# zkemail/halo2-regex

Hardware: AMD Instinct MI355X
Metric: DFA witness rows/sec (higher is better)
Workload: dtype u8

## Files before the change

### halo2_regex_amd/csrc/hrx_api.cpp

```cpp
#include <fstream>
#include <sstream>

#include "hrx_ctx.hpp"
#include "hrx_fr.h"
#include "hrx_host_walk.hpp"
#include "hrx_lane.h"

using namespace hrx;

static thread_local std::string g_err;
int hrx::set_last_error(int code, const std::string &msg) {
    g_err = msg;
    return code;
}

namespace hrx {
uint32_t debug_flags_from_env() {
    const char *dbg = std::getenv("HRX_DEBUG_FLAGS");
    return dbg ? ((uint32_t)std::strtoul(dbg, nullptr, 0) & kDbgHonoured) : 0u;
}
bool match_via_rows_from_env() {
    const char *dbg = std::getenv("HRX_DEBUG_FLAGS");
    return dbg && (std::strtoull(dbg, nullptr, 0) & kDbgMatchViaRows) != 0;
}
// ... 142 lines not shown
    return table_endpoint_rows(defs->s, d, rows3, cap_rows);
}


int hrx_device_count(int *count) {
    if (!count) return fail(HRX_ERR_ARG, "NULL argument");
    *count = 0;
    HIP_TRY(hipGetDeviceCount(count));
    return HRX_OK;
}

void hrx_shard_range(size_t B, int world, int rank, size_t *begin, size_t *count) {
    if (world < 1) world = 1;
    const size_t per = (B + (size_t)world - 1) / (size_t)world;
    size_t b = per * (size_t)rank;
    if (b > B) b = B;
    size_t e = b + per;
    if (e > B) e = B;
    if (begin) *begin = b;
    if (count) *count = e - b;
}

static int ctx_create_from(const DefsSet &set, int device, hrx_ctx **out);

int hrx_ctx_create(const hrx_defs *defs, int device, hrx_ctx **out) {
    if (!defs || !out) return fail(HRX_ERR_ARG, "NULL argument");
    if (!defs->s.finalized) return fail(HRX_ERR_STATE, "call hrx_defs_finalize first");
    return ctx_create_from(defs->s, device, out);
}

int hrx_ctx_clone(const hrx_ctx *ctx, int device, hrx_ctx **out) {
    if (!ctx || !out) return fail(HRX_ERR_ARG, "NULL argument");
    hrx_ctx *c = nullptr;
    const int rc = ctx_create_from(ctx->s, device == HRX_DEVICE_SAME ? ctx->device : device, &c);
    if (rc != HRX_OK) return rc;
    c->host_threshold = ctx->host_threshold;
    c->tune = ctx->tune;
    c->match_fused_wide = ctx->match_fused_wide;
    c->place_dry = ctx->place_dry; c->host_route = ctx->host_route; c->host_threads = ctx->host_threads; c->host_pipeline = ctx->host_pipeline; c->host_chunk_mib = ctx->host_chunk_mib; c->host_trace = ctx->host_trace;
    c->place_enabled = ctx->place_enabled; c->place_max_bytes = ctx->place_max_bytes; c->place_max_ms = ctx->place_max_ms;
    *out = c;
    return HRX_OK;
}

static int ctx_create_from(const DefsSet &set, int device, hrx_ctx **out) {
    struct { const DefsSet &s; } defs_view{set};
    const auto *defs = &defs_view;
    if (device == HRX_DEVICE_NONE) {
        hrx_ctx *c = new hrx_ctx();
        c->s = defs->s;
        c->device = HRX_DEVICE_NONE;
        c->debug = debug_flags_from_env();
        c->match_via_rows = match_via_rows_from_env();
        *out = c;
        return HRX_OK;
    }
    int count = 0;
    HIP_TRY(hipGetDeviceCount(&count));
    if (device < 0 || device >= count) return fail(HRX_ERR_ARG, "no such device");
    DeviceGuard guard;
    HIP_TRY(guard.set(device));
    hipDeviceProp_t prop;
    HIP_TRY(hipGetDeviceProperties(&prop, device));
    if (std::strncmp(prop.gcnArchName, "gfx950", 6) != 0)
        return fail(HRX_ERR_HIP, std::string("kernels are built for gfx950 only; device is ") + prop.gcnArchName);
    hrx_ctx *c = new hrx_ctx();
    c->s = defs->s;
    c->device = device;
    c->num_cus = prop.multiProcessorCount;
    c->debug = debug_flags_from_env();
    c->match_via_rows = match_via_rows_from_env();
    if (const char *v = std::getenv("HRX_HOST_PIPELINE")) c->host_pipeline = std::atoi(v) != 0 ? 1 : 2;
    if (const char *v = std::getenv("HRX_HOST_CHUNK_MIB")) { const long n = std::atol(v); if (n >= 4 && n <= 4096) c->host_chunk_mib = (size_t)n; }
    if (const char *v = std::getenv("HRX_HOST_TRACE")) c->host_trace = std::atoi(v) != 0;
    if (const char *v = std::getenv("HRX_PLACE")) c->place_enabled = std::atoi(v) != 0;
    if (const char *v = std::getenv("HRX_MP_COMBINE")) c->mp_combine = std::atoi(v) != 0;
    if (const char *v = std::getenv("HRX_PLACE_TRACE")) c->place_trace = std::atoi(v) != 0;
    if (const char *v = std::getenv("HRX_PLACE_MAX_STEPS")) { const int n = std::atoi(v); if (n >= 1 && n <= 256) { c->place_max_steps = n; c->place_max_steps_set = true; } }
    c->pool = pool_acquire(device);
    hipError_t e = hipStreamCreateWithFlags(&c->stream, hipStreamNonBlocking);
    if (e == hipSuccess) e = hipStreamCreateWithFlags(&c->copy_stream, hipStreamNonBlocking);
    if (e == hipSuccess) e = hipMalloc((void **)&c->d_group_counter, 64);
    if (e == hipSuccess) e = hipMemset(c->d_group_counter, 0, 64);

    if (c->s.groups.empty()) {
        if (e == hipSuccess) e = upload_images(c->s, c->d_table, c->d_wide, c->d_half, c->d_pairtab);
        if (e == hipSuccess) e = upload_blob(c->s.byte.image, c->d_bytetab);
    } else {
        c->groups.resize(c->s.groups.size());
        for (size_t g = 0; e == hipSuccess && g < c->s.groups.size(); ++g) {
            e = upload_images(c->s.groups[g], c->groups[g].d_table, c->groups[g].d_wide, c->groups[g].d_half, c->groups[g].d_pairtab);
            if (e == hipSuccess) e = upload_blob(c->s.groups[g].byte.image, c->groups[g].d_bytetab);
        }
    }
    c->cw_groups.resize(c->s.cw_groups.size());
    for (size_t g = 0; e == hipSuccess && g < c->s.cw_groups.size(); ++g) {
        e = c->cw_groups[g].d_cw.reserve(c->s.cw_groups[g].cw_image.size());
        if (e == hipSuccess) e = hipMemcpy(c->cw_groups[g].d_cw.p, c->s.cw_groups[g].cw_image.data(), c->s.cw_groups[g].cw_image.size(), hipMemcpyHostToDevice);
    }
    if (e == hipSuccess && !c->s.cw_image.empty()) {
        e = c->d_cw.reserve(c->s.cw_image.size());
        if (e == hipSuccess) e = hipMemcpy(c->d_cw.p, c->s.cw_image.data(), c->s.cw_image.size(), hipMemcpyHostToDevice);
    }
    for (size_t d = 0; e == hipSuccess && d < c->s.pair_tags.size(); ++d) {
        uint16_t *p = nullptr;
        e = hipMalloc((void **)&p, c->s.pair_tags[d].size() * 2);
        if (e == hipSuccess) {
            c->d_pair.push_back(p);
            e = hipMemcpy(p, c->s.pair_tags[d].data(), c->s.pair_tags[d].size() * 2, hipMemcpyHostToDevice);
        }
    }
    for (size_t d = 0; e == hipSuccess && d < c->s.endpoint_member.size(); ++d) {
        uint8_t *p = nullptr;
        e = hipMalloc((void **)&p, c->s.endpoint_member[d].size());
        if (e == hipSuccess) {
            c->d_member.push_back(p);
            e = hipMemcpy(p, c->s.endpoint_member[d].data(), c->s.endpoint_member[d].size(), hipMemcpyHostToDevice);
        }
    }
    if (e != hipSuccess) {
        hrx_ctx_destroy(c);
        return fail(HRX_ERR_HIP, std::string("ctx setup: ") + hipGetErrorString(e));
    }
    *out = c;
    return HRX_OK;
}

int hrx_ctx_set_host_threshold(hrx_ctx *ctx, size_t rows) {
    if (!ctx) return fail(HRX_ERR_ARG, "NULL ctx");
    std::lock_guard<std::mutex> lk(ctx->mu);
    ctx->host_threshold = rows;
    return HRX_OK;
}

size_t hrx_ctx_host_threshold(const hrx_ctx *ctx) { return ctx ? ctx->host_threshold : 0; }
int hrx_ctx_device(const hrx_ctx *ctx) { return ctx ? ctx->device : HRX_DEVICE_NONE; }

void hrx_ctx_destroy(hrx_ctx *c) {
    if (!c) return;
    DeviceGuard guard;
    if (c->device != HRX_DEVICE_NONE) (void)guard.set(c->device);
    if (c->stream) { (void)hipStreamSynchronize(c->stream); (void)hipStreamDestroy(c->stream); }
    if (c->copy_stream) { (void)hipStreamSynchronize(c->copy_stream); (void)hipStreamDestroy(c->copy_stream); }
    if (c->d_table) (void)hipFree(c->d_table);
    if (c->d_wide) (void)hipFree(c->d_wide);
    if (c->d_half) (void)hipFree(c->d_half);
    if (c->d_pairtab) (void)hipFree(c->d_pairtab);
    if (c->d_bytetab) (void)hipFree(c->d_bytetab);
    for (auto &g : c->groups) {
        if (g.d_table) (void)hipFree(g.d_table);
        if (g.d_wide) (void)hipFree(g.d_wide);
        if (g.d_half) (void)hipFree(g.d_half);
        if (g.d_pairtab) (void)hipFree(g.d_pairtab);
        if (g.d_bytetab) (void)hipFree(g.d_bytetab);
        g.records.release(); g.status.release(); g.summary.release();
    }
    c->mp_masked.release(); c->mp_ov.release();
    c->tp_records.release(); c->tp_masked.release();
    c->spec_cimage.release(); c->d_cw.release(); c->verify_img.dev.release(); c->lookup_img.dev.release(); c->compress_img.dev.release();
    for (auto &g : c->cw_groups) { g.d_cw.release(); g.status.release(); g.summary.release(); }
    c->spec_cls.release(); c->spec_ends.release(); c->spec_fail.release(); c->spec_init.release(); c->spec_vstatus.release(); c->spec_vinfo.release(); c->spec_work.release();
    if (c->d_group_counter) (void)hipFree(c->d_group_counter);
    pool_release(c->pool);
#ifdef HRX_STAMPS
    c->stamps.release();
#endif
    for (uint16_t *p : c->d_pair) (void)hipFree(p);
    for (uint8_t *p : c->d_member) (void)hipFree(p);
    c->chars.release(); c->lens.release(); c->records.release(); c->masked.release();
    c->status.release(); c->states.release(); c->tags.release();
    c->match_rec.release(); c->match_msk.release(); c->match_chars.release(); c->match_counts.release(); c->match_spans.release(); c->match_lens.release(); c->match_status.release();
    delete c;
}


}

namespace {

struct BatchIo {
    const uint8_t *chars;
    size_t stride;
    const uint32_t *lens;
    size_t B, M;
    hipStream_t st;
    uint32_t *const *planes;
    size_t n_planes;
};
struct PassOut {
    int layout;
    uint32_t *records;
    uint16_t *masked;
    uint64_t *status;
    size_t rec_pitch, msk_pitch;
    uint32_t rec_D = 0;
    uint32_t *summary = nullptr;
    uint32_t merge_G = 0;
    const uint32_t *const *merge_summary = nullptr;
    uint32_t *merge_ov = nullptr;
};

SetImages device_images(const hrx_ctx *c) { return {c->d_table, c->d_wide, c->d_half, c->d_pairtab, c->d_bytetab, nullptr}; }
SetImages device_images(const hrx_ctx::GroupDev &g) { return {g.d_table, g.d_wide, g.d_half, g.d_pairtab, g.d_bytetab, nullptr}; }
SetImages class_wide_images(const DevBuf &d_cw) { SetImages im; im.cw = (const uint8_t *)d_cw.p; return im; }

int claim_scratch(hrx_ctx *ctx, hipStream_t st, const char *what) {
    if (ctx->scratch_used && ctx->scratch_stream != st && hipStreamSynchronize(ctx->scratch_stream) != hipSuccess) {
        (void)hipGetLastError();
        return fail(HRX_ERR_STATE, std::string("the context's ") + what + " in use on another stream and that stream cannot be waited for here (stream capture?): one context serves one stream / graph at a time");
    }
    ctx->scratch_stream = st; ctx->scratch_used = true;
    return HRX_OK;
}

int scout_tables_ready(hrx_ctx *ctx) {
    if (ctx->spec_tables_ready) return HRX_OK;
    ctx->spec_tables = build_scout_tables(ctx->s);
    ctx->spec_cimage_bytes = 0;
    const std::vector<uint8_t> &img = ctx->spec_tables.cimage;
    if (!img.empty() && !std::getenv("HRX_SPEC_NO_COMPACT")) {
        HIP_TRY(ctx->spec_cimage.reserve(img.size()));
        HIP_TRY(hipMemcpy(ctx->spec_cimage.p, img.data(), img.size(), hipMemcpyHostToDevice));
        ctx->spec_cimage_bytes = (uint32_t)img.size();
    }
    ctx->spec_tables_ready = true;
    return HRX_OK;
}

int setup_chunks(hrx_ctx *ctx, const BatchIo &io, const DefsSet &set, const LaunchInfo &li, WitnessArgs &a, SpecArgs &sp) {
    if (&set != &ctx->s || !ctx->s.groups.empty() || ctx->d_pair.empty()) return fail(HRX_ERR_STATE, "chunked launch planned for a group of a multi-pass config");
    if (int rc = claim_scratch(ctx, io.st, "chunk scratch is")) return rc;
    if (int rc = scout_tables_ready(ctx)) return rc;
    const uint32_t C = (uint32_t)li.spec_chunks, Dn = a.D, G = li.n_groups;
    const size_t B = io.B, Bpad = (size_t)G * 64;
    uint32_t smax = 4;
    for (uint32_t d = 0; d < Dn; ++d) smax = std::max<uint32_t>(smax, (uint32_t)set.defs[d].allstr.largest_state_val + 1);
    smax = (smax + 15u) & ~15u;
    const uint32_t row_bytes = smax + 32u;
    HIP_TRY(ctx->spec_cls.reserve((size_t)C * Dn * Bpad * row_bytes));
    HIP_TRY(ctx->spec_init.reserve((size_t)C * B * Dn * 4));
    HIP_TRY(ctx->spec_vstatus.reserve((size_t)C * B * 8));
    HIP_TRY(ctx->spec_vinfo.reserve((size_t)C * B * 8));
    HIP_TRY(ctx->spec_work.reserve(16 + (size_t)C * B * 8));
    sp.chars = io.chars; sp.stride = io.stride; sp.lens = io.lens; sp.B = (uint32_t)B; sp.M = (uint32_t)io.M; sp.D = Dn; sp.in_pm = (a.layout & HRX_LAYOUT_INPUT_POSITION_MAJOR) ? 1u : 0u;
    sp.C = C; sp.tiles_per_chunk = (uint32_t)li.spec_tiles; sp.n_groups = G;
// ... 225 lines not shown
    const size_t Dn = ctx->s.defs.size();
    if (!record_planes || !(n_planes == Dn || (Dn == 1 && n_planes == 2))) return fail(HRX_ERR_ARG, "record planes: one buffer per RegexDefs of the config (one def: one buffer, or two row stripes)");
    for (size_t d = 0; d < n_planes; ++d)
        if ((B && !record_planes[d]) || ((uintptr_t)record_planes[d] & 15)) return fail(HRX_ERR_ARG, "record planes must be 16-byte aligned device buffers");
    std::lock_guard<std::mutex> lk(ctx->mu);
    DeviceGuard guard;
    if (ctx->device != HRX_DEVICE_NONE) HIP_TRY(guard.set(ctx->device));
    return launch_batch(ctx, chars, stride, lens, B, M, record_planes[0], masked, status, (hipStream_t)stream, 0, 0, layout, n_planes > 1 ? record_planes : nullptr, n_planes);
}

int hrx_ctx_set_option(hrx_ctx *ctx, int option, long value) {
    if (!ctx) return fail(HRX_ERR_ARG, "NULL ctx");
    std::lock_guard<std::mutex> lk(ctx->mu);
    switch (option) {
        case HRX_OPT_PMD_COMBINER_WAVE:
            if (value < 0 || value > 2) return fail(HRX_ERR_ARG, "HRX_OPT_PMD_COMBINER_WAVE: 0 (default), 1 (on) or 2 (off)");
            ctx->tune = (ctx->tune & ~kTunePmdFinMask) | (uint32_t)value;
            return HRX_OK;
        case HRX_OPT_HOST_ROUTE:
            if (value < 0 || value > 2) return fail(HRX_ERR_ARG, "HRX_OPT_HOST_ROUTE: HRX_HOST_ROUTE_AUTO, _DEVICE or _HOST");
            ctx->host_route = (int)value;
            return HRX_OK;
        case HRX_OPT_HOST_THREADS:
            if (value < 0 || value > 4096) return fail(HRX_ERR_ARG, "HRX_OPT_HOST_THREADS: 0 (the calling thread's cores) .. 4096");
            ctx->host_threads = (int)value;
            return HRX_OK;
        case HRX_OPT_HOST_PIPELINE:
            if (value < 0 || value > 2) return fail(HRX_ERR_ARG, "HRX_OPT_HOST_PIPELINE: 0 (measured), 1 (pipelined) or 2 (one stream)");
            ctx->host_pipeline = (int)value;
            return HRX_OK;
        case HRX_OPT_PLACE_DRY_LAUNCH:
            if (value < 0 || value > 1) return fail(HRX_ERR_ARG, "HRX_OPT_PLACE_DRY_LAUNCH: 0 or 1");
            ctx->place_dry = value != 0;
            return HRX_OK;
        case HRX_OPT_MATCH_FUSED_WIDE:
            if (value < 0 || value > 1) return fail(HRX_ERR_ARG, "HRX_OPT_MATCH_FUSED_WIDE: 0 or 1");
            ctx->match_fused_wide = value != 0;
            return HRX_OK;
        default: return fail(HRX_ERR_ARG, "hrx_ctx_set_option: unknown option");
    }
}

long hrx_ctx_get_option(const hrx_ctx *ctx, int option) {
    if (!ctx) return -1;
    switch (option) {
        case HRX_OPT_PMD_COMBINER_WAVE: return (long)(ctx->tune & kTunePmdFinMask);
        case HRX_OPT_HOST_ROUTE: return ctx->host_route;
        case HRX_OPT_HOST_THREADS: return ctx->host_threads;
        case HRX_OPT_HOST_PIPELINE: return ctx->host_pipeline;
        case HRX_OPT_PLACE_DRY_LAUNCH: return ctx->place_dry ? 1 : 0;
        case HRX_OPT_MATCH_FUSED_WIDE: return ctx->match_fused_wide ? 1 : 0;
        default: return -1;
    }
}

size_t hrx_fr_num_columns(size_t D) { return 4 + 4 * D; }

void hrx_fr_from_u64(uint64_t v, int flags, uint64_t *limbs) {
    uint64_t w[4];
    if (v >> 32) {
        fr_from_u64(v, w, (flags & HRX_FR_CANONICAL) != 0);
    } else {
        fr_store_cell(w, fr_from_u32((uint32_t)v, (flags & HRX_FR_CANONICAL) != 0));
    }
    if (limbs) { limbs[0] = w[0]; limbs[1] = w[1]; limbs[2] = w[2]; limbs[3] = w[3]; }
}

static int fr_columns_any(hrx_ctx *ctx, int layout, const uint8_t *chars, size_t stride, const uint32_t *lens, const uint32_t *records, const uint32_t *const *planes, size_t n_planes,
                          size_t rec_pitch, const uint16_t *masked, size_t msk_pitch, size_t B, size_t M, size_t b_begin, size_t b_count, uint64_t *cells, int flags, void *stream);

int hrx_fr_columns_device(hrx_ctx *ctx, int layout, const uint8_t *chars, size_t stride, const uint32_t *lens,
                          const uint32_t *records, size_t rec_pitch, const uint16_t *masked, size_t msk_pitch, size_t B,
                          size_t M, size_t b_begin, size_t b_count, uint64_t *cells, int flags, void *stream) {
    return fr_columns_any(ctx, layout, chars, stride, lens, records, nullptr, 0, rec_pitch, masked, msk_pitch, B, M, b_begin, b_count, cells, flags, stream);
}

int hrx_fr_columns_device_planes(hrx_ctx *ctx, int layout, const uint8_t *chars, size_t stride, const uint32_t *lens, const uint32_t *const *record_planes, size_t n_planes,
                                 const uint16_t *masked, size_t B, size_t M, size_t b_begin, size_t b_count, uint64_t *cells, int flags, void *stream) {
    if (!ctx) return fail(HRX_ERR_ARG, "NULL ctx");
    if (int rc = check_rows_planes(ctx, layout, record_planes, n_planes)) return rc;
    return fr_columns_any(ctx, layout, chars, stride, lens, nullptr, record_planes, n_planes, 0, masked, 0, B, M, b_begin, b_count, cells, flags, stream);
}

static int fr_columns_any(hrx_ctx *ctx, int layout, const uint8_t *chars, size_t stride, const uint32_t *lens, const uint32_t *records, const uint32_t *const *planes, size_t n_planes,
                          size_t rec_pitch, const uint16_t *masked, size_t msk_pitch, size_t B, size_t M, size_t b_begin, size_t b_count, uint64_t *cells, int flags, void *stream) {
    if (!ctx) return fail(HRX_ERR_ARG, "NULL ctx");
    if (b_count == 0) return HRX_OK;
    if (!chars || !lens || (!records && !planes) || !masked || !cells) return fail(HRX_ERR_ARG, "NULL buffer");
    if (int rc = check_window(B, b_begin, b_count)) return rc;
    if (M == 0 || M > kRowsMaxRows || B > 0xffffffffull - 64) return fail(HRX_ERR_ARG, "shape out of range");
    if (int rc = check_rows_layout(layout)) return rc;
    if ((uintptr_t)cells & 15) return fail(HRX_ERR_ARG, "cells must be 16-byte aligned");
    if (ctx->device == HRX_DEVICE_NONE) return fail(HRX_ERR_HIP, "host-only context (HRX_DEVICE_NONE): no device to launch on");
    std::lock_guard<std::mutex> lk(ctx->mu);
    DeviceGuard guard;
    HIP_TRY(guard.set(ctx->device));
    FrArgs a{};
    a.chars = chars; a.stride = stride; a.lens = lens; a.records = records; a.masked = masked;
    for (size_t d = 0; planes && d < n_planes; ++d) a.planes[d] = planes[d];
    a.n_stripes = planes && n_planes == 2 * ctx->s.defs.size() ? 2u : 1u;
    a.B = (uint32_t)B; a.M = (uint32_t)M; a.D = (uint32_t)ctx->s.defs.size(); a.layout = (uint32_t)layout;
    a.rec_pitch = rec_pitch ? rec_pitch : M; a.msk_pitch = msk_pitch ? msk_pitch : M;
    a.canonical = (flags & HRX_FR_CANONICAL) ? 1u : 0u;
    const size_t total = b_count;
    for (size_t done = 0; done < total; done += 32768) {
        const size_t nb = total - done < 32768 ? total - done : 32768;
        a.b_begin = (uint32_t)(b_begin + done); a.b_count = (uint32_t)nb;
        a.cells = cells + done * M * 4;
        a.col_cells = total * M;
        HIP_TRY(launch_fr_columns(a, (hipStream_t)stream));
    }
    return HRX_OK;
}
int hrx_chars_to_position_major_device(hrx_ctx *ctx, const uint8_t *chars, size_t stride, size_t B, uint8_t *chars_pm, void *stream) {
    if (!ctx) return fail(HRX_ERR_ARG, "NULL ctx");
    if (ctx->device == HRX_DEVICE_NONE) return fail(HRX_ERR_HIP, "host-only context (HRX_DEVICE_NONE): no device to launch on");
    if (B == 0) return HRX_OK;
    if (!chars || !chars_pm) return fail(HRX_ERR_ARG, "NULL buffer");
    if (B > 0xffffffffull - 64 || stride / 16 > 0xffffffffull) return fail(HRX_ERR_ARG, "shape out of range");
    if ((stride & 15) || stride < 16 || ((uintptr_t)chars & 15) || ((uintptr_t)chars_pm & 15))
        return fail(HRX_ERR_ARG, "buffers must be 16-byte aligned with stride % 16 == 0 and stride >= 16");
    if (chars == chars_pm) return fail(HRX_ERR_ARG, "in-place conversion is not supported");
    DeviceGuard guard;
    HIP_TRY(guard.set(ctx->device));
    HIP_TRY(launch_chars_to_position_major(chars, stride, B, chars_pm, (hipStream_t)stream));
    return HRX_OK;
}

void hrx_position_major_plane_sizes(size_t B, size_t M, size_t *plane_u32, size_t *masked_u16) {
    if (plane_u32) *plane_u32 = (M + 3) / 4 * B * 4;
    if (masked_u16) *masked_u16 = (M + 7) / 8 * B * 8;
}

static bool rows_of_string_shape(size_t B, size_t M, size_t D, size_t b) {
    return b < B && B <= 0xffffffffull - 64 && M != 0 && M <= kRowsMaxRows && D != 0 && D <= HRX_MAX_DEFS;
}

int hrx_rows_of_string_planes(const uint32_t *const *record_planes, size_t n_planes, const uint16_t *masked_pm, size_t B, size_t M, size_t D, size_t b, uint32_t *records, uint16_t *masked) {
    if (!record_planes && !masked_pm) return fail(HRX_ERR_ARG, "NULL buffer");
    if ((record_planes && !records) || (masked_pm && !masked)) return fail(HRX_ERR_ARG, "NULL output");
    if (!rows_of_string_shape(B, M, D, b)) return fail(HRX_ERR_ARG, "string index or shape out of range");
    if (record_planes && !(n_planes == D || (D == 1 && n_planes == 2))) return fail(HRX_ERR_ARG, "one buffer per def (one def: one buffer or two row stripes)");
    if (record_planes) {
        for (size_t p = 0; p < n_planes; ++p)
            if (!record_planes[p]) return fail(HRX_ERR_ARG, "NULL plane");
        const size_t R = n_planes / D, q4 = (M + 3) / 4;
        RowsIn a{};
        a.B = (uint32_t)B; a.M = (uint32_t)(4 * ((q4 + R - 1) / R)); a.D = 1u; a.layout = HRX_LAYOUT_POSITION_MAJOR; a.n_stripes = 1u;
        for (size_t d = 0; d < D; ++d)
            for (size_t p = 0; p < R; ++p) {
                a.records = record_planes[p * D + d];
                const RowsPlace s = rows_place<false>(a, (uint32_t)b);
                for (size_t q = p; q < q4; q += R) {
                    const uint32_t *src = rec_quad<kRecPm>(a, s, (uint32_t)(q / R), 0u);
                    const size_t rows = std::min<size_t>(4, M - 4 * q);
                    for (size_t i = 0; i < rows; ++i) records[(4 * q + i) * D + d] = src[i];
                }
            }
    }
    if (masked_pm) return hrx_rows_of_string_position_major(nullptr, masked_pm, B, M, D, b, nullptr, masked);
    return HRX_OK;
}

int hrx_rows_of_string_position_major(const uint32_t *records_pm, const uint16_t *masked_pm, size_t B, size_t M, size_t D, size_t b, uint32_t *records, uint16_t *masked) {
    if (!records_pm && !masked_pm) return fail(HRX_ERR_ARG, "NULL buffer");
    if ((records_pm && !records) || (masked_pm && !masked)) return fail(HRX_ERR_ARG, "NULL output");
    if (!rows_of_string_shape(B, M, D, b)) return fail(HRX_ERR_ARG, "string index or shape out of range");
    RowsIn a{};
    a.records = records_pm; a.masked = masked_pm;
    a.B = (uint32_t)B; a.M = (uint32_t)M; a.D = (uint32_t)D; a.layout = HRX_LAYOUT_POSITION_MAJOR; a.n_stripes = 1u;
    const RowsPlace s = masked_pm ? rows_place<true>(a, (uint32_t)b) : rows_place<false>(a, (uint32_t)b);
    for (size_t q = 0; records_pm && q < (M + 3) / 4; ++q) {
        const size_t rows = std::min<size_t>(4, M - 4 * q);
        for (size_t d = 0; d < D; ++d) {
            const uint32_t *src = rec_quad<kRecPm>(a, s, (uint32_t)q, (uint32_t)d);
            for (size_t i = 0; i < rows; ++i) records[(4 * q + i) * D + d] = src[i];
        }
    }
    for (size_t o = 0; masked_pm && o < (M + 7) / 8; ++o) std::memcpy(masked + 8 * o, msk_octet(s, (uint32_t)o), 2 * std::min<size_t>(8, M - 8 * o));
    return HRX_OK;
}

void hrx_position_major_sizes(size_t B, size_t M, size_t D, size_t *records_u32, size_t *masked_u16) {
    if (records_u32) *records_u32 = (M + 3) / 4 * B * 4 * D;
    if (masked_u16) *masked_u16 = (M + 7) / 8 * B * 8;
}

void hrx_recommended_pitches(size_t M, size_t *rec_pitch, size_t *msk_pitch, size_t *chars_stride) {
    const size_t m64 = (M + 63) / 64 * 64;
    if (rec_pitch) *rec_pitch = m64 + 32;
    if (msk_pitch) *msk_pitch = m64 + 64;
    if (chars_stride) *chars_stride = (M + 127) / 128 * 128 + 128;
}
// ... 4 lines not shown
```

### halo2_regex_amd/csrc/hrx_ctx.hpp

```cpp
#pragma once
#include <hip/hip_runtime_api.h>

#include <algorithm>
#include <atomic>
#include <chrono>
#include <cstdarg>
#include <cstdio>
#include <cstdlib>
#include <cstring>
#include <map>
#include <mutex>
#include <string>
#include <thread>
#include <vector>

#include "../../include/hrx.h"
#include "hrx_defs.hpp"
#include "hrx_error.hpp"
#include "hrx_plan.hpp"
#include "hrx_rows.hpp"

namespace hrx { struct VerifyDefRows; struct LookupRun; }

#define HRX_INTERNAL __attribute__((visibility("hidden")))
// ... 33 lines not shown
        const size_t want = bytes + bytes / 4 + 4096;
        hipError_t e = hipMalloc(&p, want);
        if (e == hipSuccess) cap = want;
        return e;
    }
    void release() { if (p) (void)hipFree(p); p = nullptr; cap = 0; }
};


struct CtxImage {
    std::vector<uint32_t> host;
    DevBuf dev;
};

struct hrx_place_arena;
struct hrx_place_pool;
HRX_INTERNAL void arena_retire(hrx_place_arena *a);
HRX_INTERNAL hrx_place_pool *pool_acquire(int device);
HRX_INTERNAL void pool_release(hrx_place_pool *p);

struct hrx_ctx {
    hrx::DefsSet s;
    int device = 0;
    int num_cus = 0;
    uint32_t debug = 0;
    uint32_t tune = 0;
    size_t host_threshold = HRX_DEFAULT_HOST_THRESHOLD;
    hipStream_t stream = nullptr;
    struct HostMode { unsigned calls = 0, until_probe = 0; bool sequential = false; double piped_ns_per_byte = 0.0, seq_ns_per_byte = 0.0; } host_mode;
    int host_route = 0, host_threads = 0, host_pipeline = 0;
    size_t host_chunk_mib = 48;
    bool host_trace = false;
    struct HostRates { double dev_alone = 0.0, host_alone = 0.0, split_total = 0.0, dev_ns_per_row = 0.0, host_ns_per_row = 0.0; unsigned calls = 0; } host_rates;
    hrx_host_route_report last_host{};
    hipStream_t copy_stream = nullptr;
    uint32_t *d_table = nullptr;
    uint64_t *d_wide = nullptr;
    uint16_t *d_half = nullptr;
    uint8_t *d_pairtab = nullptr;
    uint8_t *d_bytetab = nullptr;
    std::vector<uint16_t *> d_pair;
    std::vector<uint8_t *> d_member;
    std::mutex mu;
    DevBuf chars, lens, records, masked, status, states, tags;
    struct GroupDev {
        uint32_t *d_table = nullptr;
        uint64_t *d_wide = nullptr;
        uint16_t *d_half = nullptr;
        uint8_t *d_pairtab = nullptr;
        uint8_t *d_bytetab = nullptr;
        DevBuf records, status, summary;
    };
    std::vector<GroupDev> groups;
    struct CwGroupDev { DevBuf d_cw, status, summary; };
    std::vector<CwGroupDev> cw_groups;
    DevBuf mp_masked;
    DevBuf mp_ov;
    bool mp_combine = false;
    DevBuf tp_records, tp_masked;
    DevBuf spec_cls, spec_ends, spec_fail, spec_init, spec_vstatus, spec_vinfo, spec_work;
    bool spec_tables_ready = false;
    hrx::ScoutTables spec_tables;
    DevBuf spec_cimage;
    uint32_t spec_cimage_bytes = 0;
    uint32_t *d_group_counter = nullptr;
    hipStream_t scratch_stream = nullptr;
    bool scratch_used = false;
    bool place_enabled = true, place_trace = false, place_dry = true;
    int place_max_steps = 48;
    bool place_max_steps_set = false;
    double place_seen_rate = 0.0;
    size_t place_max_bytes = 0;
    double place_max_ms = 0.0;
    hrx_place_report last_place{};
    struct hrx_place_pool *pool = nullptr;
    bool match_via_rows = false;
    bool match_fused_wide = false;
    DevBuf match_rec, match_msk, match_chars, match_counts, match_spans;
    DevBuf match_lens;
    DevBuf match_status;
    hipStream_t match_stream = nullptr;
    bool match_used = false;
    CtxImage verify_img, lookup_img, compress_img;
    DevBuf d_cw;
#ifdef HRX_STAMPS
    DevBuf stamps;
#endif
};


extern "C" HRX_INTERNAL int describe_config(const hrx::DefsSet &s, const uint32_t dbg, const uint32_t tune, const bool mpc_on, int layout, size_t B, size_t M, int num_cus, char *out, size_t cap);
HRX_INTERNAL int check_host_shape(size_t B, size_t M);
HRX_INTERNAL int launch_batch(hrx_ctx *ctx, const uint8_t *chars, size_t stride, const uint32_t *lens, size_t B, size_t M, uint32_t *records, uint16_t *masked, uint64_t *status,
                              hipStream_t st, size_t rec_pitch = 0, size_t msk_pitch = 0, int layout = 0, uint32_t *const *planes = nullptr, size_t n_planes = 0);
HRX_INTERNAL int batch_host_locked(hrx_ctx *ctx, const uint8_t *chars, size_t stride, const uint32_t *lens, size_t B, size_t M, uint32_t *records, uint16_t *masked, uint64_t *status,
                                   bool one_stream = false);
HRX_INTERNAL int check_rows_layout(int layout);
HRX_INTERNAL int check_rows_planes(const hrx_ctx *ctx, int layout, const uint32_t *const *planes, size_t n_planes);
HRX_INTERNAL int check_rows(const hrx_ctx *ctx, const hrx::RowsCall &c, bool device, hrx::RowsIn &a);
HRX_INTERNAL int check_window(size_t B, size_t b_begin, size_t b_count);
HRX_INTERNAL int check_has_device(const hrx_ctx *ctx);
HRX_INTERNAL unsigned ctx_host_threads(hrx_ctx *ctx);
HRX_INTERNAL bool defs_lookup_run(const hrx::DefsSet &s, hrx::LookupRun &run);
using CtxImageBuilder = bool (*)(const hrx::VerifyDefRows *rows, size_t D, std::vector<uint32_t> &img);
HRX_INTERNAL int ctx_image_host(hrx_ctx *ctx, CtxImage &im, CtxImageBuilder build, const char *noun);
HRX_INTERNAL int ctx_image_device(hrx_ctx *ctx, CtxImage &im, CtxImageBuilder build, const char *noun, void *stream);
```

### halo2_regex_amd/csrc/hrx_kernel.hip

```cpp
#include <hip/hip_runtime.h>

#include "hrx_fr_device.h"
#include "hrx_kernel.hpp"
#include "hrx_lane.h"

namespace hrx {

__global__ void zero_u32_kernel(uint32_t *p) { *p = 0u; }
hipError_t launch_zero_u32(uint32_t *p, hipStream_t stream) {
    hipLaunchKernelGGL(zero_u32_kernel, dim3(1), dim3(1), 0, stream, p);
    return hipGetLastError();
}

hipError_t launch_witness(const WitnessArgs &a, const LaunchInfo &li, hipStream_t stream) {
    if (li.kernel == Kernel::Pp) return launch_witness_pp(a, li, stream);
    if (li.kernel == Kernel::Pmd) return launch_witness_pmd(a, li, stream);
    return li.kernel == Kernel::Pm ? launch_witness_pm(a, li, stream) : launch_witness_sm(a, li, stream);
}

struct PairArgs {
    const uint64_t *states;
    uint64_t n;
    const uint16_t *pt;
    uint32_t ns;
    uint16_t *tags;
};

__global__ void pair_tags_kernel(const PairArgs a) {
    const uint64_t r = (uint64_t)blockIdx.x * blockDim.x + threadIdx.x;
    if (r >= a.n) return;
    const uint64_t cur = a.states[r], next = a.states[r + 1];
    uint16_t t = 0;
    if (cur < a.ns && next < a.ns) t = a.pt[cur * a.ns + next];
    a.tags[r] = t;
}

hipError_t launch_pair_tags(const uint64_t *states, size_t n, uint32_t D, const uint16_t *const *pair_tags,
                            const uint32_t *n_states, uint16_t *tags, hipStream_t stream) {
    if (n == 0) return hipSuccess;
    for (uint32_t d = 0; d < D; ++d) {
        PairArgs a{states + (size_t)d * (n + 1), n, pair_tags[d], n_states[d], tags + (size_t)d * n};
        hipLaunchKernelGGL(pair_tags_kernel, dim3((unsigned)((n + 255) / 256)), dim3(256), 0, stream, a);
    }
    return hipGetLastError();
}

struct EndpointDefArgs {
    const uint64_t *states, *substr_ids;
    uint64_t n;
    const uint8_t *member;
    uint32_t n_states, n_substrs, id_offset;
    uint8_t *flags;
};

__global__ void endpoint_flags_kernel(const EndpointDefArgs a) {
    const uint64_t r = (uint64_t)blockIdx.x * blockDim.x + threadIdx.x;
    if (r >= a.n) return;
    const uint64_t sid = a.substr_ids[r];
    uint8_t f = 0;
    if (sid != 0) {
        const uint64_t j = sid - a.id_offset;
        const uint64_t cur = a.states[r], next = a.states[r + 1];
        if (j < a.n_substrs) {
            if (cur < a.n_states) f |= a.member[j * a.n_states + cur] & 1;
            if (next < a.n_states) f |= a.member[j * a.n_states + next] & 2;
        }
    }
    a.flags[r] = f;
}

hipError_t launch_endpoint_flags(const EndpointArgs &a, const uint8_t *const *member, const uint32_t *dims, hipStream_t stream) {
    if (a.n == 0) return hipSuccess;
    for (uint32_t d = 0; d < a.D; ++d) {
        EndpointDefArgs e{a.states + (size_t)d * (a.n + 1), a.substr_ids + (size_t)d * a.n, a.n, member[d], dims[3 * d], dims[3 * d + 1], dims[3 * d + 2],
                          a.flags + (size_t)d * a.n};
        hipLaunchKernelGGL(endpoint_flags_kernel, dim3((unsigned)((a.n + 255) / 256)), dim3(256), 0, stream, e);
    }
    return hipGetLastError();
}

constexpr uint32_t kFrJ = 4u;
constexpr uint32_t kFrRowsPerBlock = 4u * 32u * kFrJ;
__global__ __launch_bounds__(256) void fr_columns_kernel(const FrArgs a) {
    __shared__ uint4 frtab[512];
    fr_store16(&frtab[2u * threadIdx.x], fr_from_u32(threadIdx.x, a.canonical != 0));
    __syncthreads();
    const uint32_t half = threadIdx.x & 1u;
    const uint32_t bi = blockIdx.y;
    const uint32_t b = a.b_begin + bi;
    const uint32_t n = min(a.lens[b], a.M);
    const RowsPlace s = rows_place<true>(a, b);
    const int form = rows_form(a);
    const uint32_t wave = threadIdx.x >> 6, lane = threadIdx.x & 63u;
    const uint32_t rbase = blockIdx.x * kFrRowsPerBlock + wave * (32u * kFrJ) + (lane >> 1);
    const size_t col_cells = (size_t)a.col_cells;
    uint64_t *out0 = a.cells + ((size_t)bi * a.M + rbase) * 4u + half * 2u;
    auto put_rows = [&](const uint32_t col, const uint32_t (&v)[kFrJ]) {
#pragma unroll
        for (uint32_t j = 0; j < kFrJ; ++j) {
            if (rbase + j * 32u < a.M) {
                uint4 cell;
                if (v[j] < 256u) {
                    cell = frtab[2u * v[j] + half];
                } else {
                    const Fr w = fr_from_u32(v[j], a.canonical != 0);
                    cell = half ? fr_hi16(w) : fr_lo16(w);
                }
                unsigned char *p = reinterpret_cast<unsigned char *>(out0 + (size_t)col * col_cells * 4u + (size_t)j * 32u * 4u);
                store16_nt(p, cell);
            }
        }
    };
    uint32_t live[kFrJ], c[kFrJ];
#pragma unroll
    for (uint32_t j = 0; j < kFrJ; ++j) {
        const uint32_t r = min(rbase + j * 32u, a.M - 1u);
        live[j] = (rbase + j * 32u) < n ? 1u : 0u;
        c[j] = 0;
        if (live[j]) c[j] = chr_cell(s, r);
    }
    put_rows(0, live);
    put_rows(1, c);
    for (uint32_t d = 0; d < a.D; ++d) {
        uint32_t rec[kFrJ], f[kFrJ];
#pragma unroll
        for (uint32_t j = 0; j < kFrJ; ++j) {
            const uint32_t r = min(rbase + j * 32u, a.M - 1u);
            rec[j] = form == kRecPlanes ? rec_cell<kRecPlanes>(a, s, r, d) : form == kRecPm ? rec_cell<kRecPm>(a, s, r, d) : rec_cell<kRecSm>(a, s, r, d);
        }
#pragma unroll
        for (uint32_t j = 0; j < kFrJ; ++j) f[j] = rec[j] & 0xffffu;
        put_rows(2 + 4 * d, f);
#pragma unroll
        for (uint32_t j = 0; j < kFrJ; ++j) f[j] = (rec[j] >> 16) & 0xffu;
        put_rows(3 + 4 * d, f);
#pragma unroll
        for (uint32_t j = 0; j < kFrJ; ++j) f[j] = (rec[j] >> 24) & 1u;
        put_rows(4 + 4 * d, f);
#pragma unroll
        for (uint32_t j = 0; j < kFrJ; ++j) f[j] = (rec[j] >> 25) & 1u;
        put_rows(5 + 4 * d, f);
    }
    uint32_t mk[kFrJ], f[kFrJ];
#pragma unroll
    for (uint32_t j = 0; j < kFrJ; ++j) {
        const uint32_t r = min(rbase + j * 32u, a.M - 1u);
        mk[j] = form == kRecSm ? msk_cell<false>(s, r) : msk_cell<true>(s, r);
    }
#pragma unroll
    for (uint32_t j = 0; j < kFrJ; ++j) f[j] = mk[j] & 0xffu;
    put_rows(2 + 4 * a.D, f);
#pragma unroll
    for (uint32_t j = 0; j < kFrJ; ++j) f[j] = mk[j] >> 8;
    put_rows(3 + 4 * a.D, f);
}

hipError_t launch_fr_columns(const FrArgs &a, hipStream_t stream) {
    if (a.b_count == 0 || a.M == 0) return hipSuccess;
    hipLaunchKernelGGL(fr_columns_kernel, dim3((a.M + kFrRowsPerBlock - 1u) / kFrRowsPerBlock, a.b_count), dim3(256), 0, stream, a);
    return hipGetLastError();
}

}
```

### halo2_regex_amd/csrc/hrx_kernel.hpp

```cpp
#pragma once
#include <hip/hip_runtime_api.h>

#include <cstddef>
#include <cstdint>

#include "hrx_defs.hpp"
#include "hrx_extract.hpp"
#include "hrx_route.hpp"
#include "hrx_rows.hpp"

namespace hrx {

struct LaunchInfo;
struct WitnessArgs;
constexpr uint32_t kMaxDefsPerLaunch = 8;

struct WitnessArgs {
    const uint8_t *chars;
    uint64_t stride;
    const uint32_t *lens;
    uint32_t B, M;
    uint32_t rec_pitch, msk_pitch;
    uint32_t layout;
    uint32_t *records;
// ... 238 lines not shown
    uint64_t base;
};
hipError_t launch_match_ragged(const RaggedMatchArgs &r, const MatchPlan &p, int num_cus, hipStream_t stream);
hipError_t launch_ragged_slice(const uint8_t *values, const uint64_t *offsets, uint64_t base, size_t b0, size_t n, uint32_t limit, size_t stride,
                               uint8_t *out, uint32_t *lens, hipStream_t stream);
hipError_t launch_ragged_to_position_major(const uint8_t *values, const uint64_t *offsets, uint64_t base, size_t B, size_t stride, uint8_t *chars_pm,
                                           uint32_t *lens, hipStream_t stream);

struct SelectedSrc {
    const uint8_t *src;
    const uint64_t *offsets;
    const uint32_t *lens;
    uint64_t src_stride;
};
hipError_t launch_match_selected(const MatchArgs &a, const SelectedSrc &s, const uint32_t *sel, size_t n_sel, const MatchPlan &p, int num_cus,
                                 hipStream_t stream);
hipError_t launch_selected_slice(const SelectedSrc &s, size_t B, const uint32_t *sel, size_t k0, size_t n, uint32_t limit, size_t stride, uint8_t *out,
                                 uint32_t *lens, hipStream_t stream);
struct SpanScatter {
    const uint32_t *sel;
    uint32_t B_src;
    uint64_t *status;
    uint32_t *span_counts;
    uint64_t *spans;
};
hipError_t launch_spans_from_masked_selected(const MatchArgs &a, const SpanScatter &o, hipStream_t stream);
struct MatchWideArgs;
hipError_t launch_match_wide(const MatchWideArgs &a, const SelectedSrc &s, uint64_t base, const uint32_t *sel, size_t n_sel, const MatchPlan &p, int num_cus,
                             hipStream_t stream);

constexpr uint32_t kExtractThreads = 256;
struct ExtractArgs {
    ExtractIn in;
    uint64_t *run_offsets;
    uint64_t *runs;
    uint64_t *byte_offsets;
    uint8_t *values;
    uint64_t *totals;
    uint64_t runs_cap, values_cap;
    uint64_t *ws;
};
size_t extract_workspace_bytes(size_t B);
hipError_t launch_extract(const ExtractArgs &a, hipStream_t stream);

struct RouteArgs {
    RouteIn in;
    uint32_t *order;
    uint64_t *bucket_offsets;
    uint64_t *ws;
};
size_t route_workspace_bytes(size_t B);
hipError_t launch_route(const RouteArgs &a, hipStream_t stream);
hipError_t launch_gather_to_position_major(const uint8_t *src, size_t src_stride, const uint32_t *lens, const uint64_t *offsets, size_t B,
                                           const uint32_t *sel, size_t n_sel, size_t stride, uint8_t *chars_pm, uint32_t *lens_out, hipStream_t stream);

struct TransposeArgs {
    const uint32_t *records_pm;
    const uint16_t *masked_pm;
    uint32_t B, M, D;
    uint32_t *records;
    uint16_t *masked;
    uint32_t rec_pitch, msk_pitch;
};
hipError_t launch_transpose(const TransposeArgs &a, hipStream_t stream);
hipError_t launch_chars_to_position_major(const uint8_t *chars_sm, size_t stride, size_t B, uint8_t *chars_pm, hipStream_t stream);

hipError_t launch_pair_tags(const uint64_t *states, size_t n, uint32_t D, const uint16_t *const *pair_tags,
                            const uint32_t *n_states, uint16_t *tags, hipStream_t stream);

struct EndpointArgs {
    const uint64_t *states;
    const uint64_t *substr_ids;
    uint64_t n;
    uint32_t D;
    uint8_t *flags;
};
hipError_t launch_endpoint_flags(const EndpointArgs &a, const uint8_t *const *member, const uint32_t *dims, hipStream_t stream);

struct FrArgs : RowsIn {
    uint32_t b_begin, b_count;
    uint32_t canonical;
    uint64_t *cells;
    uint64_t col_cells;
};
hipError_t launch_fr_columns(const FrArgs &a, hipStream_t stream);

struct VerifyArgs;
hipError_t launch_verify_rows(const VerifyArgs &a, hipStream_t stream);
struct VerifyChunkArgs;
hipError_t launch_verify_chunked(const VerifyChunkArgs &ca, hipStream_t stream);
struct LookupArgs;
hipError_t launch_lookup_counts(const LookupArgs &a, size_t lds_bytes, hipStream_t stream);
struct CompressArgs;
struct CompressTableArgs;
hipError_t launch_compress_inputs(const CompressArgs &a, hipStream_t stream);
hipError_t launch_compress_table(const CompressTableArgs &a, hipStream_t stream);
struct PermuteArgs;
hipError_t launch_lookup_permute(const PermuteArgs &a, hipStream_t stream);
struct InvertArgs;
struct ProductArgs;
hipError_t launch_lookup_invert(const InvertArgs &a, hipStream_t stream);
hipError_t launch_lookup_product(const ProductArgs &a, hipStream_t stream);
struct NttArgs;
hipError_t launch_ntt_prepare(uint32_t k, uint32_t *ws, hipStream_t stream);
hipError_t launch_ntt(const NttArgs &a, int device, hipStream_t stream);
struct QuotientArgs;
struct VanishArgs;
hipError_t launch_lookup_quotient(const QuotientArgs &a, hipStream_t stream);
hipError_t launch_vanishing_inverse(const VanishArgs &a, hipStream_t stream);

}
```

Baseline: 871.7 billion.

## Make Fr column kernel persistent with per-context precomputed Fr table

Replaces the one-block-per-row-tile grid of the Fr columns kernel with a persistent grid sized to CUs times five workgroups. Each wave walks contiguous row runs across batch entries and writes one column at a time, so stores stream sequentially into each column plane. The 0..255 Fr lookup table is now computed once per context by a separate kernel and copied into LDS, instead of every block running the field conversion. The cost is more per-element work: a column-descriptor switch on each pass, and the record and mask words are re-read for every derived column rather than once per definition.

```diff
diff --git a/halo2_regex_amd/csrc/hrx_api.cpp b/halo2_regex_amd/csrc/hrx_api.cpp
--- a/halo2_regex_amd/csrc/hrx_api.cpp
+++ b/halo2_regex_amd/csrc/hrx_api.cpp
@@ -248,6 +248,7 @@
     if (e == hipSuccess) e = hipStreamCreateWithFlags(&c->copy_stream, hipStreamNonBlocking);
     if (e == hipSuccess) e = hipMalloc((void **)&c->d_group_counter, 64);
     if (e == hipSuccess) e = hipMemset(c->d_group_counter, 0, 64);
+    if (e == hipSuccess) e = hipMalloc(&c->d_fr_table, kFrTableBytes);
 
     if (c->s.groups.empty()) {
         if (e == hipSuccess) e = upload_images(c->s, c->d_table, c->d_wide, c->d_half, c->d_pairtab);
@@ -327,6 +328,7 @@
     for (auto &g : c->cw_groups) { g.d_cw.release(); g.status.release(); g.summary.release(); }
     c->spec_cls.release(); c->spec_ends.release(); c->spec_fail.release(); c->spec_init.release(); c->spec_vstatus.release(); c->spec_vinfo.release(); c->spec_work.release();
     if (c->d_group_counter) (void)hipFree(c->d_group_counter);
+    if (c->d_fr_table) (void)hipFree(c->d_fr_table);
     pool_release(c->pool);
 #ifdef HRX_STAMPS
     c->stamps.release();
@@ -718,6 +720,23 @@
     return fr_columns_any(ctx, layout, chars, stride, lens, nullptr, record_planes, n_planes, 0, masked, 0, B, M, b_begin, b_count, cells, flags, stream);
 }
 
+static int fr_table_ready(hrx_ctx *ctx, hipStream_t st) {
+    if (ctx->fr_table_filled) {
+        if (ctx->fr_table_waited || ctx->fr_table_stream == st) return HRX_OK;
+        if (hipStreamSynchronize(ctx->fr_table_stream) != hipSuccess) {
+            (void)hipGetLastError();
+            return fail(HRX_ERR_STATE, "the context's Fr table was filled on another stream and that stream cannot be waited for here (stream capture?)");
+        }
+        ctx->fr_table_waited = true;
+        return HRX_OK;
+    }
+    hipStreamCaptureStatus cap = hipStreamCaptureStatusNone;
+    if (hipStreamIsCapturing(st, &cap) != hipSuccess) { (void)hipGetLastError(); cap = hipStreamCaptureStatusNone; }
+    HIP_TRY(launch_fr_table(ctx->d_fr_table, st));
+    if (cap == hipStreamCaptureStatusNone) { ctx->fr_table_filled = true; ctx->fr_table_stream = st; }
+    return HRX_OK;
+}
+
 static int fr_columns_any(hrx_ctx *ctx, int layout, const uint8_t *chars, size_t stride, const uint32_t *lens, const uint32_t *records, const uint32_t *const *planes, size_t n_planes,
                           size_t rec_pitch, const uint16_t *masked, size_t msk_pitch, size_t B, size_t M, size_t b_begin, size_t b_count, uint64_t *cells, int flags, void *stream) {
     if (!ctx) return fail(HRX_ERR_ARG, "NULL ctx");
@@ -738,13 +757,15 @@
     a.B = (uint32_t)B; a.M = (uint32_t)M; a.D = (uint32_t)ctx->s.defs.size(); a.layout = (uint32_t)layout;
     a.rec_pitch = rec_pitch ? rec_pitch : M; a.msk_pitch = msk_pitch ? msk_pitch : M;
     a.canonical = (flags & HRX_FR_CANONICAL) ? 1u : 0u;
+    if (int rc = fr_table_ready(ctx, (hipStream_t)stream)) return rc;
+    a.fr_table = ctx->d_fr_table;
     const size_t total = b_count;
     for (size_t done = 0; done < total; done += 32768) {
         const size_t nb = total - done < 32768 ? total - done : 32768;
         a.b_begin = (uint32_t)(b_begin + done); a.b_count = (uint32_t)nb;
         a.cells = cells + done * M * 4;
         a.col_cells = total * M;
-        HIP_TRY(launch_fr_columns(a, (hipStream_t)stream));
+        HIP_TRY(launch_fr_columns(a, ctx->num_cus, (hipStream_t)stream));
     }
     return HRX_OK;
 }
diff --git a/halo2_regex_amd/csrc/hrx_ctx.hpp b/halo2_regex_amd/csrc/hrx_ctx.hpp
--- a/halo2_regex_amd/csrc/hrx_ctx.hpp
+++ b/halo2_regex_amd/csrc/hrx_ctx.hpp
@@ -139,6 +139,10 @@
     hipStream_t match_stream = nullptr;
     bool match_used = false;
     CtxImage verify_img, lookup_img, compress_img;
+    void *d_fr_table = nullptr;
+    bool fr_table_filled = false;
+    hipStream_t fr_table_stream = nullptr;
+    bool fr_table_waited = false;
     DevBuf d_cw;
 #ifdef HRX_STAMPS
     DevBuf stamps;
diff --git a/halo2_regex_amd/csrc/hrx_kernel.hip b/halo2_regex_amd/csrc/hrx_kernel.hip
--- a/halo2_regex_amd/csrc/hrx_kernel.hip
+++ b/halo2_regex_amd/csrc/hrx_kernel.hip
@@ -1,4 +1,6 @@
 #include <hip/hip_runtime.h>
+
+#include <cstdlib>
 
 #include "hrx_fr_device.h"
 #include "hrx_kernel.hpp"
@@ -79,85 +81,115 @@
     return hipGetLastError();
 }
 
-constexpr uint32_t kFrJ = 4u;
-constexpr uint32_t kFrRowsPerBlock = 4u * 32u * kFrJ;
-__global__ __launch_bounds__(256) void fr_columns_kernel(const FrArgs a) {
-    __shared__ uint4 frtab[512];
-    fr_store16(&frtab[2u * threadIdx.x], fr_from_u32(threadIdx.x, a.canonical != 0));
-    __syncthreads();
-    const uint32_t half = threadIdx.x & 1u;
-    const uint32_t bi = blockIdx.y;
-    const uint32_t b = a.b_begin + bi;
-    const uint32_t n = min(a.lens[b], a.M);
-    const RowsPlace s = rows_place<true>(a, b);
-    const int form = rows_form(a);
-    const uint32_t wave = threadIdx.x >> 6, lane = threadIdx.x & 63u;
-    const uint32_t rbase = blockIdx.x * kFrRowsPerBlock + wave * (32u * kFrJ) + (lane >> 1);
-    const size_t col_cells = (size_t)a.col_cells;
-    uint64_t *out0 = a.cells + ((size_t)bi * a.M + rbase) * 4u + half * 2u;
-    auto put_rows = [&](const uint32_t col, const uint32_t (&v)[kFrJ]) {
-#pragma unroll
-        for (uint32_t j = 0; j < kFrJ; ++j) {
-            if (rbase + j * 32u < a.M) {
-                uint4 cell;
-                if (v[j] < 256u) {
-                    cell = frtab[2u * v[j] + half];
-                } else {
-                    const Fr w = fr_from_u32(v[j], a.canonical != 0);
-                    cell = half ? fr_hi16(w) : fr_lo16(w);
-                }
-                unsigned char *p = reinterpret_cast<unsigned char *>(out0 + (size_t)col * col_cells * 4u + (size_t)j * 32u * 4u);
-                store16_nt(p, cell);
-            }
-        }
-    };
-    uint32_t live[kFrJ], c[kFrJ];
-#pragma unroll
-    for (uint32_t j = 0; j < kFrJ; ++j) {
-        const uint32_t r = min(rbase + j * 32u, a.M - 1u);
-        live[j] = (rbase + j * 32u) < n ? 1u : 0u;
-        c[j] = 0;
-        if (live[j]) c[j] = chr_cell(s, r);
-    }
-    put_rows(0, live);
-    put_rows(1, c);
-    for (uint32_t d = 0; d < a.D; ++d) {
-        uint32_t rec[kFrJ], f[kFrJ];
-#pragma unroll
-        for (uint32_t j = 0; j < kFrJ; ++j) {
-            const uint32_t r = min(rbase + j * 32u, a.M - 1u);
-            rec[j] = form == kRecPlanes ? rec_cell<kRecPlanes>(a, s, r, d) : form == kRecPm ? rec_cell<kRecPm>(a, s, r, d) : rec_cell<kRecSm>(a, s, r, d);
-        }
-#pragma unroll
-        for (uint32_t j = 0; j < kFrJ; ++j) f[j] = rec[j] & 0xffffu;
-        put_rows(2 + 4 * d, f);
-#pragma unroll
-        for (uint32_t j = 0; j < kFrJ; ++j) f[j] = (rec[j] >> 16) & 0xffu;
-        put_rows(3 + 4 * d, f);
-#pragma unroll
-        for (uint32_t j = 0; j < kFrJ; ++j) f[j] = (rec[j] >> 24) & 1u;
-        put_rows(4 + 4 * d, f);
-#pragma unroll
-        for (uint32_t j = 0; j < kFrJ; ++j) f[j] = (rec[j] >> 25) & 1u;
-        put_rows(5 + 4 * d, f);
-    }
-    uint32_t mk[kFrJ], f[kFrJ];
-#pragma unroll
-    for (uint32_t j = 0; j < kFrJ; ++j) {
-        const uint32_t r = min(rbase + j * 32u, a.M - 1u);
-        mk[j] = form == kRecSm ? msk_cell<false>(s, r) : msk_cell<true>(s, r);
-    }
-#pragma unroll
-    for (uint32_t j = 0; j < kFrJ; ++j) f[j] = mk[j] & 0xffu;
-    put_rows(2 + 4 * a.D, f);
-#pragma unroll
-    for (uint32_t j = 0; j < kFrJ; ++j) f[j] = mk[j] >> 8;
-    put_rows(3 + 4 * a.D, f);
+__global__ __launch_bounds__(256) void fr_table_kernel(uint4 *tab) {
+    fr_store16(&tab[2u * threadIdx.x], fr_from_u32(threadIdx.x, false));
+    fr_store16(&tab[512u + 2u * threadIdx.x], fr_from_u32(threadIdx.x, true));
+}
+hipError_t launch_fr_table(void *tab, hipStream_t stream) {
+    hipLaunchKernelGGL(fr_table_kernel, dim3(1), dim3(256), 0, stream, static_cast<uint4 *>(tab));
+    return hipGetLastError();
 }
 
-hipError_t launch_fr_columns(const FrArgs &a, hipStream_t stream) {
-    if (a.b_count == 0 || a.M == 0) return hipSuccess;
-    hipLaunchKernelGGL(fr_columns_kernel, dim3((a.M + kFrRowsPerBlock - 1u) / kFrRowsPerBlock, a.b_count), dim3(256), 0, stream, a);
+constexpr uint32_t kFrJ = 4u;
+constexpr uint32_t kFrWgPerCu = 5u;
+constexpr uint32_t kFrRun = 1024u;
+
+enum : uint32_t { kFrLive, kFrChr, kFrMskSm, kFrMskPm, kFrRecSm, kFrRecPm, kFrRecPlanes };
+struct FrColumn { uint32_t src, d, shift, mask; };
+__device__ __forceinline__ FrColumn fr_column(const uint32_t col, const uint32_t D, const int form) {
+    if (col < 2u) return {col ? kFrChr : kFrLive, 0u, 0u, 0xffu};
+    if (col >= 2u + 4u * D) return {form == kRecSm ? kFrMskSm : kFrMskPm, 0u, col == 2u + 4u * D ? 0u : 8u, 0xffu};
+    const uint32_t f = (col - 2u) & 3u;
+    return {form == kRecSm ? kFrRecSm : form == kRecPm ? kFrRecPm : kFrRecPlanes, (col - 2u) >> 2, f == 0u ? 0u : f == 1u ? 16u : 22u + f, f == 0u ? 0xffffu : f == 1u ? 0xffu : 1u};
+}
+
+template <uint32_t CPP>
+__global__ __launch_bounds__(256) void fr_columns_kernel(const FrArgs a) {
+    const uint32_t run = a.run, runs = (a.M + run - 1u) / run;
+    if ((uint64_t)blockIdx.x * 4u >= (uint64_t)a.b_count * runs) return;
+    __shared__ uint4 frtab[512];
+    const uint4 *tab = static_cast<const uint4 *>(a.fr_table) + (a.canonical ? 512u : 0u);
+    frtab[threadIdx.x] = tab[threadIdx.x];
+    frtab[256u + threadIdx.x] = tab[256u + threadIdx.x];
+    __syncthreads();
+    const uint32_t half = threadIdx.x & 1u, row = (threadIdx.x & 63u) >> 1;
+    const uint32_t w = blockIdx.x * 4u + (threadIdx.x >> 6), W = gridDim.x * 4u;
+    const uint32_t dq = W / runs, dr = W % runs;
+    const int form = rows_form(a);
+    const uint32_t ncols = 4u + 4u * a.D, cpp = CPP ? CPP : ncols;
+    for (uint32_t c0 = 0; c0 < ncols; c0 += cpp) {
+        for (uint32_t bi = w / runs, k = w % runs; bi < a.b_count;) {
+            const uint32_t b = a.b_begin + bi;
+            const RowsPlace s = rows_place<true>(a, b);
+            const uint32_t n = c0 < 2u ? min(a.lens[b], a.M) : 0u;
+            const uint32_t r0 = k * run, rend = min(r0 + run, a.M);
+            for (uint32_t col = c0; col < c0 + cpp; ++col) {
+                const FrColumn fc = fr_column(col, a.D, form);
+                uint64_t *out = a.cells + ((size_t)col * a.col_cells + (size_t)bi * a.M) * 4u + half * 2u;
+                for (uint32_t rb = r0; rb < rend; rb += 32u * kFrJ) {
+                    uint32_t v[kFrJ], r[kFrJ];
+#pragma unroll
+                    for (uint32_t j = 0; j < kFrJ; ++j) r[j] = min(rb + j * 32u + row, a.M - 1u);
+                    switch (fc.src) {
+#define HRX_FR_READ(expr)                                          \
+    _Pragma("unroll") for (uint32_t j = 0; j < kFrJ; ++j) v[j] = (expr); \
+    break
+                        case kFrLive: HRX_FR_READ(r[j] < n ? 1u : 0u);
+                        case kFrChr: HRX_FR_READ(r[j] < n ? chr_cell(s, r[j]) : 0u);
+                        case kFrMskSm: HRX_FR_READ(msk_cell<false>(s, r[j]));
+                        case kFrMskPm: HRX_FR_READ(msk_cell<true>(s, r[j]));
+                        case kFrRecSm: HRX_FR_READ(rec_cell<kRecSm>(a, s, r[j], fc.d));
+                        case kFrRecPm: HRX_FR_READ(rec_cell<kRecPm>(a, s, r[j], fc.d));
+                        default: HRX_FR_READ(rec_cell<kRecPlanes>(a, s, r[j], fc.d));
+#undef HRX_FR_READ
+                    }
+#pragma unroll
+                    for (uint32_t j = 0; j < kFrJ; ++j) {
+                        const uint32_t x = (v[j] >> fc.shift) & fc.mask;
+                        if (rb + j * 32u + row < a.M) {
+                            uint4 cell;
+                            if (x < 256u) {
+                                cell = frtab[2u * x + half];
+                            } else {
+                                const Fr f = fr_from_u32(x, a.canonical != 0);
+                                cell = half ? fr_hi16(f) : fr_lo16(f);
+                            }
+                            store16_nt(out + (size_t)(rb + j * 32u + row) * 4u, cell);
+                        }
+                    }
+                }
+            }
+            bi += dq; k += dr;
+            if (k >= runs) { k -= runs; ++bi; }
+        }
+    }
+}
+
+static uint32_t fr_run_of(const FrArgs &a, const uint32_t waves) {
+    uint32_t run = kFrRun;
+    while (run > 32u * kFrJ && (uint64_t)a.b_count * ((a.M + run - 1u) / run) < waves) run >>= 1;
+    return run;
+}
+
+hipError_t launch_fr_columns(const FrArgs &args, int num_cus, hipStream_t stream) {
+    if (args.b_count == 0 || args.M == 0) return hipSuccess;
+    FrArgs a = args;
+    uint32_t wgs = kFrWgPerCu;
+#ifdef HRX_FR_SWEEP
+    const char *e_cpp = std::getenv("HRX_FR_CPP"), *e_run = std::getenv("HRX_FR_RUN"), *e_wgs = std::getenv("HRX_FR_WGS");
+    if (e_wgs && std::atoi(e_wgs) >= 1 && std::atoi(e_wgs) <= 8) wgs = (uint32_t)std::atoi(e_wgs);
+#endif
+    const dim3 grid((uint32_t)num_cus * wgs);
+    a.run = fr_run_of(a, grid.x * 4u);
+#ifdef HRX_FR_SWEEP
+    if (e_run) a.run = std::atoi(e_run) > 0 ? ((uint32_t)std::atoi(e_run) + 32u * kFrJ - 1u) / (32u * kFrJ) * (32u * kFrJ) : (a.M + 32u * kFrJ - 1u) / (32u * kFrJ) * (32u * kFrJ);
+    const uint32_t cpp = e_cpp ? (uint32_t)std::atoi(e_cpp) : 0u;
+    if (cpp == 1u) hipLaunchKernelGGL((fr_columns_kernel<1u>), grid, dim3(256), 0, stream, a);
+    else if (cpp == 2u) hipLaunchKernelGGL((fr_columns_kernel<2u>), grid, dim3(256), 0, stream, a);
+    else if (cpp == 4u) hipLaunchKernelGGL((fr_columns_kernel<4u>), grid, dim3(256), 0, stream, a);
+    else
+#endif
+    hipLaunchKernelGGL((fr_columns_kernel<0u>), grid, dim3(256), 0, stream, a);
     return hipGetLastError();
 }
 
diff --git a/halo2_regex_amd/csrc/hrx_kernel.hpp b/halo2_regex_amd/csrc/hrx_kernel.hpp
--- a/halo2_regex_amd/csrc/hrx_kernel.hpp
+++ b/halo2_regex_amd/csrc/hrx_kernel.hpp
@@ -344,8 +344,12 @@
     uint32_t canonical;
     uint64_t *cells;
     uint64_t col_cells;
-};
-hipError_t launch_fr_columns(const FrArgs &a, hipStream_t stream);
+    uint32_t run;
+    const void *fr_table;
+};
+hipError_t launch_fr_columns(const FrArgs &a, int num_cus, hipStream_t stream);
+constexpr size_t kFrTableBytes = 2u * 256u * 32u;
+hipError_t launch_fr_table(void *tab, hipStream_t stream);
 
 struct VerifyArgs;
 hipError_t launch_verify_rows(const VerifyArgs &a, hipStream_t stream);
```

New measurement: 874.0 billion, median of 2. Within noise of the previous version (+0.3%).
